# mtumalan/VisionTransformer

Measured on AMD Instinct MI355X. Metric: images/sec (512×512) ViT-B/16 seg, 1/2/4/8 MI355X + mask argmax match, higher is better.
Workload: dtype f32

## Files before the change

visiontransformer_amd/csrc/common.hpp:

```cpp
#pragma once
#include <hip/hip_runtime.h>
#include <stdint.h>

#include "../../include/vitseg.h"

namespace vitseg {

constexpr int WAVE = 64;

typedef float f32x4 __attribute__((ext_vector_type(4)));
typedef float f32x16 __attribute__((ext_vector_type(16)));
typedef short bf16x8 __attribute__((ext_vector_type(8)));
typedef short bf16x4 __attribute__((ext_vector_type(4)));

void set_error(const char* fmt, ...);
int hip_fail(hipError_t e, const char* what);

enum Opt {
    OPT_NO_F32P = 0,
    OPT_NO_P8,
    OPT_NO_H16P,
    OPT_NO_RAGGED_P8,
    OPT_NO_DROPMASK,
    OPT_DROPW_LIMIT_MB,
    OPT_UPSAMPLE_GLOBAL,
    OPT_BF16_TILES,
    OPT_F32P_NOINL,
    OPT_GN,
    OPT_NO_MASK2,
    OPT_NO_SMALL,
    OPT_SMALL_VARIANT,
    OPT_SMALL_MAX_ROWS,
    OPT_CONV_DMA,
    OPT_COUNT
};
long opt(int id);

#define VITSEG_CHECK_ARG(cond, code, ...) \
    do {                                  \
        if (!(cond)) {                    \
            ::vitseg::set_error(__VA_ARGS__); \
            return (code);                \
        }                                 \
    } while (0)

#define VITSEG_LAUNCH_CHECK(what)                               \
    do {                                                        \
        hipError_t e__ = hipGetLastError();                     \
// ... 241 lines not shown
```

visiontransformer_amd/csrc/forward.hip:

```cpp
#include "kernels.hpp"
#include "profile.hpp"
#include "forward.hpp"

namespace vitseg {

using namespace plan;

long small_max_rows() {
    const long v = opt(OPT_SMALL_MAX_ROWS);
    return v > 0 ? v : SMALL_MAX_ROWS;
}

bool small_applies(const vitseg_config* cfg, int batch, int precision) {
    Shape s;
    if (precision == VITSEG_F32X3 || opt(OPT_NO_SMALL) || check_config(cfg, &s)) return false;
    const long rows = (long)batch * s.N;
    if (!(rows < small_max_rows() && s.D % 64 == 0 && s.I % 32 == 0 && s.I > s.D && s.S % 4 == 0)) return false;
    const long lim16 = opt(OPT_SMALL_MAX_ROWS) > 0 ? opt(OPT_SMALL_MAX_ROWS) : small_max_rows_16(s.N);
    if (precision != VITSEG_F32 && !(s.I % 64 == 0 && attn_small_infer(s.Np) && rows < lim16)) return false;
    if (precision != VITSEG_F32 && ((s.D / small_splits(s.D, s.D)) % 64 || (s.I / small_splits(s.D, s.I)) % 64)) return false;
    return true;
}

namespace {
// ... 60 lines not shown
    if (!f.logits && !f.mask) return VITSEG_OK;
    const double px = (double)f.batch * s.S * s.S;
    ProfScope ps(f.prof.upsample, (f.logits ? px * s.C * 4 : 0.0) + (f.mask ? px : 0.0) + (double)f.batch * s.C * s.Np * 4, f.st);
    return launch_upsample(f.Z, f.logits, f.mask, f.batch, s.C, s.g, s.S, f.st);
}

}

int walk_large(const Fwd& f) {
    const Shape& s = f.s;
    const int Mp = f.batch * s.Np, Mt = Mp + f.batch, D = s.D, I = s.I;
    hipStream_t st = f.st;
    int rc;
    if ((rc = embed_gemm(f, f.layer(0).xin, f.h16 ? 1 : f.x3))) return rc;
    const int thin_rows = f.thin_rows ? thin_cls_rows(Mp, f.batch) : 0;
    auto gemm = [&](const void* A, int w, int b, int l, const float* R, void* C, int N, int K, int epi, int kind,
                    DropArgs dr = DropArgs{}, void* aux = nullptr) {
        GemmArgs g{};
        g.A = A; g.W = wg(f, w, l); g.bias = wt(f, b, l); g.R = R; g.C = C; g.aux = aux; g.drop = dr;
        g.M = Mt; g.N = N; g.K = K; g.lda = K; g.ldc = N;
        if (f.whole_split || thin_rows) {
            g.thin_rows = thin_rows;
            g.thin_scratch = f.scratch;
            g.thin_capacity = f.scratch_floats;
        }
        ProfScope ps(kind, 2.0 * g.M * g.N * g.K, st);
        if (f.fc1_train && epi == EPI_GELU) return launch_gemm_bf16_train(g, EPI_GELU, st);
        return f.h16 ? launch_gemm_bf16(g, A_PLAIN, epi, st, f.h16 == 2) : launch_gemm_f32(g, A_PLAIN, epi, st, f.x3);
    };
    auto lnorm = [&](const float* X, int w, int b, int l, void* H, int rows) {
        ProfScope ps(f.prof.ln, (double)rows * D * (f.h16 ? 6 : 8), st);
        return launch_layernorm(X, wt(f, w, l), wt(f, b, l), H, rows, D, f.eps, f.h16, st);
    };
    const bool mlp1 = f.prof.mlp_one_scope;
    for (int l = 0; l < s.L; ++l) {
        const LayerIO io = f.layer(l);
        if ((rc = lnorm(io.xin, VITSEG_T_LN1_W, VITSEG_T_LN1_B, l, io.h1, Mt))) return rc;
        if ((rc = gemm(io.h1, VITSEG_T_WQKV, VITSEG_T_BQKV, l, nullptr, io.qkv, 3 * D, D, EPI_BIAS, f.prof.qkv))) return rc;
        {
            ProfScope ps(f.prof.attn, 4.0 * f.batch * s.A * (double)s.N * s.N * 64, st);
            const DropArgs dr = drop(f, l, 1);
            if (io.dropw && (rc = launch_attn_dropmask((unsigned*)io.dropw, f.batch, s.Np, s.A, dr, st))) return rc;
            rc = f.h16 ? launch_attention_bf16(io.qkv, io.ctx, io.lse, f.batch, s.Np, s.A, dr, st, f.h16 == 2, io.dropw)
                       : launch_attention_f32((const float*)io.qkv, (float*)io.ctx, io.lse, f.batch, s.Np, s.A, dr, st, f.x3 != 0);
            if (rc) return rc;
        }
        if ((rc = gemm(io.ctx, VITSEG_T_WO, VITSEG_T_BO, l, io.xin, io.xmid, D, D, EPI_RESADD, f.prof.oproj, drop(f, l, 2))))
            return rc;
        if ((rc = lnorm(io.xmid, VITSEG_T_LN2_W, VITSEG_T_LN2_B, l, io.h2, Mt))) return rc;
        ProfScope ps(mlp1 ? f.prof.fc1 : -1, 4.0 * Mt * D * I, st);
        if ((rc = gemm(io.h2, VITSEG_T_W1, VITSEG_T_B1, l, nullptr, io.uact, I, D, EPI_GELU, mlp1 ? -1 : f.prof.fc1, DropArgs{},
                       io.upre)))
            return rc;
        if ((rc = gemm(io.uact, VITSEG_T_W2, VITSEG_T_B2, l, io.xmid, io.xout, D, I, EPI_RESADD, mlp1 ? -1 : f.prof.fc2,
                       drop(f, l, 3))))
            return rc;
    }
    if ((rc = lnorm(f.layer(s.L - 1).xout, VITSEG_T_LNF_W, VITSEG_T_LNF_B, 0, f.hf, Mp))) return rc;
    if ((rc = head_conv_gemm(f)) || (rc = head_1x1(f))) return rc;
    return upsample(f);
}

int walk_small(const Fwd& f) {
    const Shape& s = f.s;
    const int Mp = f.batch * s.Np, Mt = Mp + f.batch, D = s.D;
    hipStream_t st = f.st;
    float* part = f.scratch;
    const size_t dstride = (size_t)Mt * D;
    int rc;
    auto linear = [&](const void* A, int K, int w, int b, int l, void* C, int N, int epi, void* aux, int kind) {
// ... 112 lines not shown
```

visiontransformer_amd/csrc/gemm_dispatch.hip:

```cpp
#include "gemm_tiles.hpp"

namespace vitseg {
namespace {

int whole_split_shape(int M, int N, int K, int kstep) { return K % kstep == 0 ? whole_split(M, N, K, kstep) : 0; }

int thin_slices(int K, int kstep) {
    if (K < 256 || K % kstep != 0) return 0;
    const int sl = K / kstep / 4;
    return sl > THIN_MAX_SPLITS ? THIN_MAX_SPLITS : sl < 1 ? 1 : sl;
}

int whole_split_applies(const GemmArgs& a, int epi, int kstep) {
    const int sp = whole_split_shape(a.M, a.N, a.K, kstep);
    const bool ok = sp && a.thin_scratch && (size_t)sp * a.M * a.N <= a.thin_capacity && !a.drop.thresh &&
                    !a.aux && a.splitk <= 1 && a.ldc % 4 == 0 && (epi == EPI_BIAS || epi == EPI_GELU || epi == EPI_RESADD);
    return ok ? sp : 0;
}

int thin_split_applies(const GemmArgs& a, int epi, int kstep) {
    const bool h16 = kstep == 64;
    const int sl = thin_slices(a.K, kstep);
    const bool ok = sl && a.thin_scratch && a.thin_rows > 0 && a.thin_rows <= THIN_MAX_ROWS && a.M > a.thin_rows &&
                    (size_t)sl * a.thin_rows * a.N <= a.thin_capacity && (a.M - a.thin_rows) % BM == 0 &&
// ... 23 lines not shown
    int slices;
    int colsum_rows;
};

}

int launch_gemm_f32(const GemmArgs& a_in, int amode, int epi, hipStream_t s, int x3) {
    if (x3 != 1 && x3 != 2) x3 = 0;
    GemmArgs a = a_in;
    if (amode == A_PLAIN) {
        if (const int sp = whole_split_applies(a_in, epi, 32)) {
            a.thin_rows = a_in.M;
            return launch_thin_rows(GT_F32, x3, a, epi, sp, s);
        }
        if (const int sl = thin_split_applies(a_in, epi, 32)) {
            if (int rc = launch_thin_rows(GT_F32, x3, a_in, epi, sl, s)) return rc;
            a.M = a_in.M - a_in.thin_rows;
        }
    }
    a.thin_scratch = nullptr;
    VITSEG_CHECK_ARG(a.M > 0 && a.N > 0 && a.K > 0 && a.K % 4 == 0, VITSEG_EINVAL, "gemm_f32: bad M/N/K %d %d %d", a.M, a.N, a.K);
    VITSEG_CHECK_ARG(a.N % 4 == 0 && a.ldc % 4 == 0, VITSEG_ESHAPE, "gemm: N=%d and ldc=%d must be multiples of 4", a.N, a.ldc);
    if (amode == A_PLAIN) {
        VITSEG_CHECK_ARG(a.lda % 4 == 0, VITSEG_EINVAL, "gemm_f32: lda %% 4");
        if (!x3 && gemm_f32p_applies(a, epi)) return launch_gemm_f32p(a, epi, s);
    } else if (amode == A_PATCH && epi == EPI_POS) {
        VITSEG_CHECK_ARG(a.P % 4 == 0, VITSEG_ESHAPE, "patch size must be a multiple of 4");
    } else if (amode == A_CONV3 && epi == EPI_RELU) {
        VITSEG_CHECK_ARG(a.D % 4 == 0, VITSEG_ESHAPE, "hidden size must be a multiple of 4");
    }
    static const char* const who[3] = {"gemm_f32", "gemm_f32 (x3)", "gemm_f32 (x3, split W)"};
// ... 58 lines not shown
    r.body_rows = a.M;
    if (amode == A_PLAIN) {
        VITSEG_CHECK_ARG(a.lda % 8 == 0, VITSEG_EINVAL, "gemm_bf16: lda %% 8");
        r.body = xl ? HK_XL : large ? HK_LARGE : HK_TILE;
        if (epi == EPI_BIAS || epi == EPI_GELU || epi == EPI_DGELU || epi == EPI_RESADD) return VITSEG_OK;
    } else if (amode == A_CONV3 && (epi == EPI_RELU || epi == EPI_BIAS)) {
        VITSEG_CHECK_ARG(a.D % 64 == 0 && a.zeros, VITSEG_ESHAPE, "%s must be a multiple of 64",
                         epi == EPI_RELU ? "hidden size" : "channel count");
        r.body = large ? HK_LARGE : HK_TILE;
        return VITSEG_OK;
    }
    set_error("gemm_bf16: unsupported amode/epilogue %d/%d", amode, epi);
    return VITSEG_EINVAL;
}

int launch_gemm_bf16(const GemmArgs& a_in, int amode, int epi, hipStream_t s, bool f16) {
    H16Route r;
    if (int rc = route_h16(a_in, amode, epi, r)) return rc;
    const GemmType type = f16 ? GT_F16 : GT_BF16;
    const bool out_f32 = epi == EPI_RESADD || amode == A_CONV3;
    GemmArgs a = a_in;
    if (r.slices) {
        a.thin_rows = r.tail_rows;
        if (int rc = launch_thin_rows(type, 0, a, epi, r.slices, s)) return rc;
    }
    a.M = r.body_rows;
    a.thin_scratch = nullptr;
    if (!r.colsum_rows) a.colsum_scratch = nullptr;
    int rc = VITSEG_OK;
    switch (r.body) {
        case HK_NONE: break;
        case HK_P8: rc = launch_gemm_p8(a, epi, s, f16); break;
        case HK_H16P: rc = launch_gemm_h16p(a, s, f16); break;
        case HK_XL: rc = launch_gemm_large(f16, amode, epi, 256, a, s, "gemm_bf16"); break;
        case HK_LARGE: rc = launch_gemm_large(f16, amode, epi, 128, a, s, "gemm_bf16"); break;
        case HK_TILE: rc = launch_gemm_tile(type, out_f32, amode, epi, 0, a, s, "gemm_bf16");
    }
    if (rc) return rc;
    if (r.tail_rows && !r.slices) {
        GemmArgs t = a;
        const auto row = [&](const void* p, size_t esz) { return (char*)p + (size_t)r.body_rows * a.ldc * esz; };
        t.M = r.tail_rows;
        t.row_base = a.row_base + r.body_rows;
        t.A = (const char*)a.A + (size_t)r.body_rows * a.lda * 2;
        if (a.aux) t.aux = row(a.aux, 2);
        if (a.R) t.R = (const float*)row(a.R, epi == EPI_RESADD ? 4 : 2);
        t.C = row(a.C, out_f32 ? 4 : 2);
        if ((rc = launch_gemm_tile(type, out_f32, A_PLAIN, epi, 0, t, s, "gemm_bf16"))) return rc;
    }
    if (!a_in.colsum_out) return VITSEG_OK;
    VITSEG_CHECK_ARG(a_in.colsum_scratch && !f16, VITSEG_EINVAL, "gemm: column sums need bf16 + scratch");
    if (r.colsum_rows > 0)
        return launch_colsum_finish_fused((const bf16_t*)a_in.C + (size_t)r.colsum_rows * a_in.ldc, a_in.M - r.colsum_rows,
                                          2 * ((r.colsum_rows + 255) / 256), a_in.colsum_out, a_in.colsum_scratch, a_in.N,
// ... 40 lines not shown
```

visiontransformer_amd/csrc/gemm_tile.hip:

```cpp
#include "gemm_tiles.hpp"

namespace vitseg {
namespace {

template <typename T> struct Elem;
template <> struct Elem<float> { static constexpr int CE = 4, BKE = 32; };
template <> struct Elem<bf16_t> { static constexpr int CE = 8, BKE = 64; };
template <> struct Elem<f16_t> { static constexpr int CE = 8, BKE = 64; };

template <typename T>
struct ARow {
    const T* base;
    int y, x;
    bool valid;
};

template <typename T, int AMODE>
__device__ __forceinline__ ARow<T> make_arow(const GemmArgs& p, int m) {
    ARow<T> r;
    r.valid = m < p.M;
    r.y = r.x = 0;
    const T* A = (const T*)p.A;
    if (!r.valid) {
        r.base = A;
// ... 467 lines not shown
    else
        gemm_tile<T, OutT, AMODE, EPI, 2, 2, TA, TB, X3>(p, lds, m0, n0, (wave >> 1) * 64, (wave & 1) * 64);
}

template <typename T, typename OutT, int AMODE, int EPI, int TA = 0, int TB = 0, int X3 = 0>
int launch_one(GemmArgs a, hipStream_t s) {
    if (a.ldw == 0) a.ldw = TB ? a.N : a.K;
    if (!a.gn) a.gn = env_gn();
    const int tiles = ((a.M + BM - 1) / BM) * ((a.N + BN - 1) / BN);
    const int splits = a.splitk > 1 ? a.splitk : 1;
    hipLaunchKernelGGL((gemm_kernel<T, OutT, AMODE, EPI, TA, TB, X3>), dim3(tiles, splits), dim3(256), 0, s, a);
    VITSEG_LAUNCH_CHECK("gemm");
    return VITSEG_OK;
}

template <int EPI, typename OutT>
__global__ __launch_bounds__(256) void thin_reduce_kernel(const float* __restrict__ partial, const float* __restrict__ bias,
                                                          const float* __restrict__ R, OutT* __restrict__ C, int rows, int N,
                                                          int ldc, int splits, OutT* __restrict__ aux, DropArgs drop,
                                                          unsigned row0) {
    const int n4 = N >> 2;
    const int i = blockIdx.x * 256 + threadIdx.x;
    if (i >= rows * n4) return;
    const int r = i / n4, c = (i - r * n4) * 4;
    const size_t slab = (size_t)rows * N;
    f32x4 acc = *(const f32x4*)(partial + (size_t)r * N + c);
    for (int sIdx = 1; sIdx < splits; ++sIdx) {
        const f32x4 v = *(const f32x4*)(partial + sIdx * slab + (size_t)r * N + c);
#pragma unroll
        for (int e = 0; e < 4; ++e) acc[e] += v[e];
    }
    f32x4 b4 = {0.f, 0.f, 0.f, 0.f};
    if (bias) b4 = *(const f32x4*)(bias + c);
    f32x4 res = {0.f, 0.f, 0.f, 0.f};
    if (EPI == EPI_RESADD) res = *(const f32x4*)(R + (size_t)r * ldc + c);
    if constexpr (EPI == EPI_DGELU) {
        const uint2 d = *(const uint2*)((const OutT*)R + (size_t)r * ldc + c);
        res[0] = H16<OutT>::lo(d.x);
        res[1] = H16<OutT>::hi(d.x);
        res[2] = H16<OutT>::lo(d.y);
        res[3] = H16<OutT>::hi(d.y);
    }
    f32x4 der = {0.f, 0.f, 0.f, 0.f};
    const unsigned key = drop.thresh ? drop_key(drop.seed, drop.stream, row0 + (unsigned)r) : 0u;
#pragma unroll
    for (int e = 0; e < 4; ++e) {
// ... 13 lines not shown
    if constexpr (sizeof(OutT) == 4) {
        *(f32x4*)(C + (size_t)r * ldc + c) = acc;
    } else {
        uint2 h;
        h.x = H16<OutT>::pack2(acc[0], acc[1]);
        h.y = H16<OutT>::pack2(acc[2], acc[3]);
        *(uint2*)(C + (size_t)r * ldc + c) = h;
        if (EPI == EPI_GELU && aux) {
            h.x = H16<OutT>::pack2(der[0], der[1]);
            h.y = H16<OutT>::pack2(der[2], der[3]);
            *(uint2*)(aux + (size_t)r * ldc + c) = h;
        }
    }
}

template <typename OutT>
int launch_thin_reduce(const GemmArgs& a, int epi, int splits, hipStream_t s) {
    const int rows = a.thin_rows, body = a.M - rows;
    const int blocks = (rows * (a.N / 4) + 255) / 256;
    const float* R = nullptr;
    if (a.R) R = epi == EPI_DGELU ? (const float*)((const OutT*)a.R + (size_t)body * a.ldc) : a.R + (size_t)body * a.ldc;
    OutT* C = (OutT*)a.C + (size_t)body * a.ldc;
    OutT* aux = a.aux ? (OutT*)a.aux + (size_t)body * a.ldc : nullptr;
    const unsigned row0 = (unsigned)(a.row_base + body);
#define VITSEG_THIN(E)                                                                                                 \
    hipLaunchKernelGGL((thin_reduce_kernel<E, OutT>), dim3(blocks), dim3(256), 0, s, a.thin_scratch, a.bias, R, C, rows, \
                       a.N, a.ldc, splits, aux, a.drop, row0)
    switch (epi) {
        case EPI_BIAS: VITSEG_THIN(EPI_BIAS); break;
        case EPI_GELU: VITSEG_THIN(EPI_GELU); break;
        case EPI_DGELU:
            if constexpr (sizeof(OutT) == 4) {
                set_error("thin_reduce: dGELU epilogue is 16-bit only");
                return VITSEG_EINVAL;
            } else {
                VITSEG_THIN(EPI_DGELU);
            }
            break;
        default: VITSEG_THIN(EPI_RESADD);
    }
#undef VITSEG_THIN
    VITSEG_LAUNCH_CHECK("thin_reduce");
    return VITSEG_OK;
}

}

int launch_gemm_tile(GemmType type, bool out_f32, int amode, int epi, int x3, const GemmArgs& a, hipStream_t s, const char* who) {
#define ROW(ID, T, OutT, AMODE, EPI, X3) \
    if (type == ID && out_f32 == (sizeof(OutT) == 4) && amode == AMODE && epi == EPI && x3 == X3) return launch_one<T, OutT, AMODE, EPI, 0, 0, X3>(a, s);
#define ROW_X3(AMODE, EPI) ROW(GT_F32, float, float, AMODE, EPI, 0) ROW(GT_F32, float, float, AMODE, EPI, 1) ROW(GT_F32, float, float, AMODE, EPI, 2)
#define ROW_H16(AMODE, EPI) ROW(GT_BF16, bf16_t, bf16_t, AMODE, EPI, 0) ROW(GT_F16, f16_t, f16_t, AMODE, EPI, 0)
#define ROW_H16_F32(AMODE, EPI) ROW(GT_BF16, bf16_t, float, AMODE, EPI, 0) ROW(GT_F16, f16_t, float, AMODE, EPI, 0)
    ROW_X3(A_PLAIN, EPI_BIAS) ROW_X3(A_PLAIN, EPI_GELU) ROW_X3(A_PLAIN, EPI_RESADD) ROW(GT_F32, float, float, A_PLAIN, EPI_RELU, 0)
    ROW_X3(A_PATCH, EPI_POS) ROW_X3(A_CONV3, EPI_RELU)
    ROW_H16(A_PLAIN, EPI_BIAS) ROW_H16(A_PLAIN, EPI_GELU) ROW_H16(A_PLAIN, EPI_DGELU)
    ROW_H16_F32(A_PLAIN, EPI_RESADD) ROW_H16_F32(A_PLAIN, EPI_BIAS) ROW_H16_F32(A_CONV3, EPI_RELU) ROW_H16_F32(A_CONV3, EPI_BIAS)
// ... 18 lines not shown
    const int rows = a.thin_rows, body = a.M - rows;
    GemmArgs t = a;
    t.A = (const char*)a.A + (size_t)body * a.lda * (type == GT_F32 ? 4 : 2);
    t.M = rows;
    t.bias = nullptr;
    t.R = nullptr;
    t.C = a.thin_scratch;
    t.ldc = a.N;
    t.splitk = slices;
    t.split_stride = (size_t)rows * a.N;
    t.thin_scratch = nullptr;
    if (type != GT_F32) {
        t.aux = nullptr;
        t.drop = DropArgs{};
    }
    if (int rc = launch_gemm_tile(type, true, A_PLAIN, EPI_BIAS, x3, t, s, "gemm (K slices)")) return rc;
    if (type == GT_F32 || epi == EPI_RESADD) return launch_thin_reduce<float>(a, epi, slices, s);
    return type == GT_F16 ? launch_thin_reduce<f16_t>(a, epi, slices, s) : launch_thin_reduce<bf16_t>(a, epi, slices, s);
}

}
```

visiontransformer_amd/csrc/kernels.hpp:

```cpp
#pragma once
#include "common.hpp"

namespace vitseg {

enum AMode {
    A_PLAIN = 0,
    A_PATCH = 1,
    A_CONV3 = 2
};
enum Epi {
    EPI_BIAS = 0,
    EPI_GELU = 1,
    EPI_RESADD = 2,
    EPI_RELU = 3,
    EPI_POS = 4,
    EPI_DGELU = 5
};

struct GemmArgs {
    const void* A;
    const void* W;
    const float* bias;
    const float* R;
    void* C;
    int M, N, K;
    int lda, ldc;
    int ldw;
    void* aux;
    float* colsum_out;
    float* colsum_scratch;
    int S, P, g, Np, Cin, D;
    const void* zeros;
    int splitk;
    size_t split_stride;
    float* thin_scratch;
    size_t thin_capacity;
    int thin_rows;
    int gn;
    DropArgs drop;
    int row_base;
};

constexpr int THIN_MAX_SPLITS = 16, THIN_MAX_ROWS = 64;
inline size_t thin_scratch_floats(int max_n) { return (size_t)THIN_MAX_SPLITS * THIN_MAX_ROWS * max_n; }
inline int whole_split(int M, int N, int K, int kstep) {
    const int tiles = ((M + 127) / 128) * ((N + 127) / 128);
    if (tiles > 128 || K < 512) return 0;
    int s = K / kstep / 4;
    if (s > 8) s = 8;
    return s >= 2 ? s : 0;
}
int launch_gemm_f32(const GemmArgs& a, int amode, int epi, hipStream_t s, int x3 = 0);
int launch_gemm_f32_bwd(const GemmArgs& a, int amode, int ta, int tb, int epi, hipStream_t s);
size_t wgrad_scratch_floats(int M, int N, int K);
int launch_wgrad_f32(GemmArgs a, float* scratch, hipStream_t s);
int launch_wgrad_bf16_tt(GemmArgs a, float* scratch, hipStream_t s);
int launch_gemm_bf16_train(const GemmArgs& a, int epi, hipStream_t s);
size_t wgrad_bf16_scratch_floats(int M, int N, int K);
int wgrad_bf16_splits(int M, int N, int K, bool p8);
// ... 76 lines not shown
```

visiontransformer_amd/csrc/vitseg_api.hip:

```cpp
#include <ctype.h>
#include <stdarg.h>
#include <stdio.h>
#include <stdlib.h>
#include <strings.h>

#include <atomic>

#include <vector>

#include "kernels.hpp"
#include "profile.hpp"
#include "forward.hpp"

namespace vitseg {

static thread_local char g_err[512] = "";

void set_error(const char* fmt, ...) {
    va_list ap;
    va_start(ap, fmt);
    vsnprintf(g_err, sizeof(g_err), fmt, ap);
    va_end(ap);
}

int hip_fail(hipError_t e, const char* what) {
    set_error("%s: %s", what, hipGetErrorString(e));
    return VITSEG_EHIP;
}

static const char* const g_opt_names[OPT_COUNT] = {"no_f32p", "no_p8", "no_h16p", "no_ragged_p8", "no_dropmask",
                                                   "dropw_limit_mb", "upsample_global", "bf16_tiles", "f32p_noinl", "gn", "no_mask2", "no_small",
                                                   "small_variant", "small_max_rows", "conv_dma"};
static std::atomic<long> g_opts[OPT_COUNT];
static int opt_index(const char* name) {
    if (!name) return -1;
    for (int i = 0; i < OPT_COUNT; ++i)
        if (!strcasecmp(name, g_opt_names[i])) return i;
    return -1;
}
static long opt_parse(int id, const char* text) {
    if (id == OPT_BF16_TILES && (text[0] == 's' || text[0] == 'l' || text[0] == 'x')) return text[0] == 's' ? 1 : text[0] == 'l' ? 2 : 3;
    char* end = nullptr;
    const long v = strtol(text, &end, 10);
    if (end != text) return v;
    return (id == OPT_DROPW_LIMIT_MB || id == OPT_GN || id == OPT_SMALL_VARIANT || id == OPT_SMALL_MAX_ROWS || id == OPT_BF16_TILES) ? 0 : 1;
}
static const bool g_opts_loaded = [] {
// ... 334 lines not shown
                            int N, int K, int epilogue, int f16, int thin_rows, float* scratch, size_t scratch_floats,
                            float dropout_p, uint32_t dropout_seed, uint32_t dropout_stream, float* colsum_out,
                            float* colsum_scratch, void* stream) {
    VITSEG_CHECK_ARG(A && Wt && C, VITSEG_EINVAL, "linear_h16_ex: null pointer");
    VITSEG_CHECK_ARG(epilogue == EPI_BIAS || epilogue == EPI_GELU || epilogue == EPI_RESADD || epilogue == EPI_DGELU,
                     VITSEG_EINVAL, "linear_h16_ex: epilogue %d", epilogue);
    VITSEG_CHECK_ARG((epilogue != EPI_RESADD && epilogue != EPI_DGELU) || R, VITSEG_EINVAL, "linear_h16_ex: epilogue needs R");
    VITSEG_CHECK_ARG(dropout_p >= 0.f && dropout_p < 1.f, VITSEG_EINVAL, "linear_h16_ex: dropout_p %f", dropout_p);
    GemmArgs g{};
    g.A = A; g.W = Wt; g.bias = bias; g.R = (const float*)R; g.C = C; g.aux = aux;
    g.M = M; g.N = N; g.K = K; g.lda = K; g.ldc = N;
    if (thin_rows > 0) {
        g.thin_rows = thin_rows;
        g.thin_scratch = scratch;
        g.thin_capacity = scratch_floats;
    }
    g.drop = drop_args(dropout_p, dropout_seed, dropout_stream);
    VITSEG_CHECK_ARG(!colsum_out || (colsum_scratch && epilogue == EPI_DGELU && !f16), VITSEG_EINVAL,
                     "linear_h16_ex: column sums come with the bf16 dGELU epilogue and need scratch");
    g.colsum_out = colsum_out;
    g.colsum_scratch = colsum_out ? colsum_scratch : nullptr;
    return launch_gemm_bf16(g, A_PLAIN, epilogue, (hipStream_t)stream, f16 != 0);
}

size_t vitseg_op_colsum_scratch_floats(int M, int N) { return colsum_scratch_floats(M, N); }

size_t vitseg_op_wgrad_bf16_scratch_floats(int M, int N, int K) { return wgrad_bf16_scratch_floats(M, N, K); }

int vitseg_op_wgrad_bf16(const void* dY, const void* X, float* dW, float* scratch, const void* zeros, int M, int N, int K,
                         void* stream) {
// ... 10 lines not shown
                              float dropout_p, uint32_t dropout_seed, uint32_t dropout_stream, void* stream) {
    VITSEG_CHECK_ARG(A && Wt && C, VITSEG_EINVAL, "linear_f32_thin: null pointer");
    VITSEG_CHECK_ARG(epilogue >= 0 && epilogue <= (x3 ? 2 : 3), VITSEG_EINVAL, "linear_f32_thin: epilogue %d", epilogue);
    VITSEG_CHECK_ARG(epilogue != EPI_RESADD || R, VITSEG_EINVAL, "linear_f32_thin: residual epilogue needs R");
    VITSEG_CHECK_ARG(x3 == 0 || x3 == 1, VITSEG_EINVAL, "linear_f32_thin: x3 %d", x3);
    VITSEG_CHECK_ARG(dropout_p >= 0.f && dropout_p < 1.f, VITSEG_EINVAL, "linear_f32_thin: dropout_p %f", dropout_p);
    VITSEG_CHECK_ARG(!aux || epilogue == EPI_GELU, VITSEG_EINVAL, "linear_f32_thin: aux belongs to the GELU epilogue");
    VITSEG_CHECK_ARG(thin_rows >= 0, VITSEG_EINVAL, "linear_f32_thin: thin_rows %d", thin_rows);
    GemmArgs g{};
    g.A = A; g.W = Wt; g.bias = bias; g.R = R; g.C = C; g.aux = aux;
    g.M = M; g.N = N; g.K = K; g.lda = K; g.ldc = N;
    if (scratch && scratch_floats) {
        g.thin_rows = thin_rows;
        g.thin_scratch = scratch;
        g.thin_capacity = scratch_floats;
    }
    if (epilogue == EPI_RESADD) g.drop = drop_args(dropout_p, dropout_seed, dropout_stream);
    return launch_gemm_f32(g, A_PLAIN, epilogue, (hipStream_t)stream, x3);
}

size_t vitseg_op_wgrad_f32_scratch_floats(int M, int N, int K) { return M > 0 && N > 0 && K > 0 ? wgrad_scratch_floats(M, N, K) : 0; }

int vitseg_op_wgrad_f32(const float* dY, const float* X, float* dW, float* scratch, int M, int N, int K, void* stream) {
    VITSEG_CHECK_ARG(dY && X && dW, VITSEG_EINVAL, "wgrad_f32: null pointer");
    GemmArgs g{};
    g.A = dY; g.W = X; g.C = dW;
    g.M = M; g.N = N; g.K = K; g.lda = M; g.ldw = N; g.ldc = N;
    return launch_wgrad_f32(g, scratch, (hipStream_t)stream);
}

// ... 218 lines not shown
```

visiontransformer_amd/csrc/vitseg_train.hip:

```cpp
#include <stdlib.h>

#include <mutex>

#include "kernels.hpp"
#include "profile.hpp"
#include "forward.hpp"

using namespace vitseg;
using namespace vitseg::plan;

namespace {

struct LayerBufs {
    size_t xin, h1, qkv, ctx, lse, xmid, h2, upre, uact;
    size_t dropw;
};
constexpr size_t DROPW_KEEP_LIMIT = (size_t)4 << 30;
struct TrainPlan {
    size_t Mt, Mp;
    size_t layer0, layer_stride;
    LayerBufs lb;
    size_t xfinal, hf, f, z;
    size_t dxa, dxb, dh, dqkv, du, dctx, dvec, g, dz, df, t, wd, scratch, wscratch, ce_partial, total;
    size_t wscratch_floats;
    size_t dxc, wt, zero, dhf, Kpad;
    size_t wt_all, wt_layer;
    size_t dxm;
    size_t dropw_shared;
    bool dropw_per_layer;
    size_t pos, dpos, dpos_t;
};

TrainPlan make_train_plan(const Shape& s, int B, int precision, int g0) {
    TrainPlan p{};
    p.Mp = (size_t)B * s.Np;
    p.Mt = p.Mp + B;
    const bool lp = precision == VITSEG_BF16;
    const size_t act = lp ? 2 : 4;
    const size_t MtD = p.Mt * s.D * 4, MtI = p.Mt * (size_t)s.I * 4;
// ... 68 lines not shown
        p.dxc = take(dxc_n * 2);
        p.dhf = take(p.Mp * s.D * 4);
        p.wt = take(wide * s.D * 2);
        p.wt_layer = (size_t)s.D * (3 * s.D + s.D + 2 * (size_t)s.I);
        p.wt_all = take(p.wt_layer * s.L * 2);
        p.zero = take(256);
        size_t w = wgrad_bf16_scratch_floats(s.D, s.I, (int)p.Kpad);
        auto mx = [&](size_t v) { w = v > w ? v : w; };
        mx(wgrad_bf16_scratch_floats(s.I, s.D, (int)p.Kpad));
        mx(wgrad_bf16_scratch_floats(s.D, s.D, (int)p.Kpad));
        mx(wgrad_bf16_scratch_floats(3 * s.D, s.D, (int)p.Kpad));
        mx(wgrad_scratch_floats(MID, 9 * s.D, (int)p.Mp));
        mx(wgrad_scratch_floats(s.D, s.Kp, (int)p.Mp));
        mx(wgrad_bf16_scratch_floats(MID, 9 * s.D, (int)p.Mp));
        mx(wgrad_bf16_scratch_floats(s.D, s.Kp, (int)p.Mp));
        mx(thin_scratch_floats(s.I > 3 * s.D ? s.I : 3 * s.D));
        p.wscratch = take(w * 4);
        p.wscratch_floats = w;
    }
    if (g0 != s.g) {
        p.pos = take((size_t)s.N * s.D * 4);
        p.dpos = take((size_t)s.N * s.D * 4);
        p.dpos_t = take((size_t)s.g * g0 * s.D * 4);
    }
    p.total = off;
    return p;
}

struct Ctx {
    void* const* events = nullptr;
// ... 279 lines not shown
        };
}

void route_bf16(const Ctx& c, BwdRoute& r) {
    const Shape s = c.s;
    const int Mt = (int)c.p.Mt, Mp = (int)c.p.Mp, D = s.D, I = s.I, B = c.B;
    hipStream_t st = c.st;
    float *scratch = c.T(c.p.scratch), *wscr = c.T(c.p.wscratch);
    void *dXc = c.TV(c.p.dxc), *t = c.TV(c.p.t);
    auto tt = [=, &c](const void* dY, const void* X, float* dW, int M, int Nd, int Kd) {
        GemmArgs g = lin(dY, X, nullptr, nullptr, dW, Nd, Kd, M, Nd, Kd);
        g.ldw = Kd;
        g.zeros = c.ws + c.p.zero;
        return launch_wgrad_bf16_tt(g, wscr, st);
    };
    r.prepare = [=, &c] {
        const size_t src0[4] = {tensor_offset(c.lay, VITSEG_T_WQKV, 0), tensor_offset(c.lay, VITSEG_T_WO, 0),
                                tensor_offset(c.lay, VITSEG_T_W1, 0), tensor_offset(c.lay, VITSEG_T_W2, 0)};
        const int R4[4] = {3 * D, D, I, D}, C4[4] = {D, D, D, I};
        ProfScope ps(VITSEG_K_TRAIN_DGRAD, 0.0, st);
        return launch_transpose_layers_bf16(c.params_lp, c.TV(c.p.wt_all), src0, R4, C4, c.lay.layer_stride, s.L, st);
    };
    r.head_wgrad = [=, &c](float* dW) {
        if (int rc = launch_cast_bf16(c.T(c.p.df), dXc, (size_t)Mp * MID, st)) return rc;
        if (int rc = launch_im2col3x3_bf16(c.TV(c.p.hf), t, B, s.g, D, st)) return rc;
        return tt(dXc, t, dW, Mp, MID, 9 * D);
    };
    r.head_dgrad = [=, &c] {
        float* dHf = c.T(c.p.dhf);
        if (int rc = launch_cast_bf16(c.T(c.p.wd), c.TV(c.p.wt), (size_t)D * 9 * MID, st)) return dense(rc, nullptr);
        GemmArgs g = lin(dXc, c.TV(c.p.wt), nullptr, nullptr, dHf, Mp, D, 9 * MID, 0, D);
// ... 19 lines not shown
    r.wgrad = [=](const void* dY, const void* X, float* dW, int M, int Nd, int Kd) {
        ProfScope ps(VITSEG_K_TRAIN_WGRAD, 2.0 * M * Nd * Kd, st);
        return tt(dY, X, dW, M, Nd, Kd);
    };
    r.dgrad = [=, &c](const void* dY, int wt, int l, void* dX, int Nd, int Kd, int epi, const void* R, float* bias_grad, bool) {
        const size_t DD = (size_t)D * D;
        const size_t off = wt == VITSEG_T_WQKV ? 0 : wt == VITSEG_T_WO ? 3 * DD : wt == VITSEG_T_W1 ? 4 * DD : 4 * DD + (size_t)I * D;
        ProfScope ps(VITSEG_K_TRAIN_DGRAD, 2.0 * Mt * Nd * Kd, st);
        GemmArgs g = lin(dY, (const unsigned short*)c.TV(c.p.wt_all) + (size_t)l * c.p.wt_layer + off, nullptr, (const float*)R, dX,
                         Mt, Kd, Nd, Nd, Kd);
        g.ldw = Nd;
        if (thin_cls_rows(Mp, B)) {
            g.thin_rows = B;
            g.thin_scratch = wscr;
            g.thin_capacity = c.p.wscratch_floats;
        }
        g.colsum_out = bias_grad;
        g.colsum_scratch = bias_grad ? scratch : nullptr;
        return dense(launch_gemm_bf16_train(g, epi, st), dX);
    };
    r.attn_bwd = [=, &c](int l, const void* dCTX, void* dQKV, float* bias_grad) {
        ProfScope ps(VITSEG_K_TRAIN_ATTN_BWD, attn_flops(c, 10), st);
        if (c.dropw(l) && !c.p.dropw_per_layer)
            if (int rc = launch_attn_dropmask((unsigned*)c.dropw(l), B, s.Np, s.A, c.dr(l, 1), st)) return rc;
        return launch_attention_bwd_bf16(c.LV(l, c.p.lb.qkv), c.LV(l, c.p.lb.ctx), dCTX, c.L(l, c.p.lb.lse), c.T(c.p.dvec), dQKV,
                                         B, s.Np, s.A, c.dr(l, 1), st, c.dropw(l), bias_grad);
    };
    r.patch_wgrad = [=, &c](const float* x, float* dX, float* dW) {
        if (s.Kp % 8 == 0) {
            if (int rc = launch_cast_bf16(dX, dXc, (size_t)Mp * D, st)) return rc;
// ... 216 lines not shown
```

Baseline: 612.4.

## Fuse thin-row split-K GEMM with last-block reduction and skip unread CLS rows

```diff
diff --git a/visiontransformer_amd/csrc/common.hpp b/visiontransformer_amd/csrc/common.hpp
--- a/visiontransformer_amd/csrc/common.hpp
+++ b/visiontransformer_amd/csrc/common.hpp
@@ -32,6 +32,7 @@
     OPT_SMALL_VARIANT,
     OPT_SMALL_MAX_ROWS,
     OPT_CONV_DMA,
+    OPT_THIN_MODE,
     OPT_COUNT
 };
 long opt(int id);
diff --git a/visiontransformer_amd/csrc/forward.hip b/visiontransformer_amd/csrc/forward.hip
--- a/visiontransformer_amd/csrc/forward.hip
+++ b/visiontransformer_amd/csrc/forward.hip
@@ -98,8 +98,12 @@
     int rc;
     if ((rc = embed_gemm(f, f.layer(0).xin, f.h16 ? 1 : f.x3))) return rc;
     const int thin_rows = f.thin_rows ? thin_cls_rows(Mp, f.batch) : 0;
+    int thin_counters = 0;
+    if ((f.whole_split || thin_rows) && (rc = thin_counters_reset(f.scratch, f.scratch_floats, st, &thin_counters))) return rc;
+    const LayerIO io_last = f.layer(s.L - 1);
+    const bool skip_cls = thin_rows && !f.fc1_train && !io_last.lse && !io_last.upre && f.drop_p == 0.f && !(opt(OPT_THIN_MODE) & 2);
     auto gemm = [&](const void* A, int w, int b, int l, const float* R, void* C, int N, int K, int epi, int kind,
-                    DropArgs dr = DropArgs{}, void* aux = nullptr) {
+                    DropArgs dr = DropArgs{}, void* aux = nullptr, bool cls_unread = false) {
         GemmArgs g{};
         g.A = A; g.W = wg(f, w, l); g.bias = wt(f, b, l); g.R = R; g.C = C; g.aux = aux; g.drop = dr;
         g.M = Mt; g.N = N; g.K = K; g.lda = K; g.ldc = N;
@@ -107,6 +111,8 @@
             g.thin_rows = thin_rows;
             g.thin_scratch = f.scratch;
             g.thin_capacity = f.scratch_floats;
+            g.thin_counters = thin_counters;
+            g.skip_rows = cls_unread ? thin_rows : 0;
         }
         ProfScope ps(kind, 2.0 * g.M * g.N * g.K, st);
         if (f.fc1_train && epi == EPI_GELU) return launch_gemm_bf16_train(g, EPI_GELU, st);
@@ -119,6 +125,7 @@
     const bool mlp1 = f.prof.mlp_one_scope;
     for (int l = 0; l < s.L; ++l) {
         const LayerIO io = f.layer(l);
+        const bool skip = skip_cls && l == s.L - 1;
         if ((rc = lnorm(io.xin, VITSEG_T_LN1_W, VITSEG_T_LN1_B, l, io.h1, Mt))) return rc;
         if ((rc = gemm(io.h1, VITSEG_T_WQKV, VITSEG_T_BQKV, l, nullptr, io.qkv, 3 * D, D, EPI_BIAS, f.prof.qkv))) return rc;
         {
@@ -129,15 +136,16 @@
                        : launch_attention_f32((const float*)io.qkv, (float*)io.ctx, io.lse, f.batch, s.Np, s.A, dr, st, f.x3 != 0);
             if (rc) return rc;
         }
-        if ((rc = gemm(io.ctx, VITSEG_T_WO, VITSEG_T_BO, l, io.xin, io.xmid, D, D, EPI_RESADD, f.prof.oproj, drop(f, l, 2))))
-            return rc;
-        if ((rc = lnorm(io.xmid, VITSEG_T_LN2_W, VITSEG_T_LN2_B, l, io.h2, Mt))) return rc;
+        if ((rc = gemm(io.ctx, VITSEG_T_WO, VITSEG_T_BO, l, io.xin, io.xmid, D, D, EPI_RESADD, f.prof.oproj, drop(f, l, 2),
+                       nullptr, skip)))
+            return rc;
+        if ((rc = lnorm(io.xmid, VITSEG_T_LN2_W, VITSEG_T_LN2_B, l, io.h2, skip ? Mp : Mt))) return rc;
         ProfScope ps(mlp1 ? f.prof.fc1 : -1, 4.0 * Mt * D * I, st);
         if ((rc = gemm(io.h2, VITSEG_T_W1, VITSEG_T_B1, l, nullptr, io.uact, I, D, EPI_GELU, mlp1 ? -1 : f.prof.fc1, DropArgs{},
-                       io.upre)))
+                       io.upre, skip)))
             return rc;
         if ((rc = gemm(io.uact, VITSEG_T_W2, VITSEG_T_B2, l, io.xmid, io.xout, D, I, EPI_RESADD, mlp1 ? -1 : f.prof.fc2,
-                       drop(f, l, 3))))
+                       drop(f, l, 3), nullptr, skip)))
             return rc;
     }
     if ((rc = lnorm(f.layer(s.L - 1).xout, VITSEG_T_LNF_W, VITSEG_T_LNF_B, 0, f.hf, Mp))) return rc;
diff --git a/visiontransformer_amd/csrc/gemm_dispatch.hip b/visiontransformer_amd/csrc/gemm_dispatch.hip
--- a/visiontransformer_amd/csrc/gemm_dispatch.hip
+++ b/visiontransformer_amd/csrc/gemm_dispatch.hip
@@ -61,7 +61,8 @@
             return launch_thin_rows(GT_F32, x3, a, epi, sp, s);
         }
         if (const int sl = thin_split_applies(a_in, epi, 32)) {
-            if (int rc = launch_thin_rows(GT_F32, x3, a_in, epi, sl, s)) return rc;
+            if (a_in.skip_rows != a_in.thin_rows)
+                if (int rc = launch_thin_rows(GT_F32, x3, a_in, epi, sl, s)) return rc;
             a.M = a_in.M - a_in.thin_rows;
         }
     }
@@ -150,13 +151,22 @@
     return VITSEG_EINVAL;
 }
 
+int thin_counters_reset(float* scratch, size_t capacity, hipStream_t s, int* lent) {
+    unsigned* cnt = (opt(OPT_THIN_MODE) & 1) ? nullptr : thin_counters_at(scratch, capacity);
+    *lent = cnt ? 1 : 0;
+    if (!cnt) return VITSEG_OK;
+    const hipError_t e = hipMemsetAsync(cnt, 0, THIN_COUNTER_WORDS * sizeof(unsigned), s);
+    return e == hipSuccess ? VITSEG_OK : hip_fail(e, "hipMemsetAsync(thin counters)");
+}
+
 int launch_gemm_bf16(const GemmArgs& a_in, int amode, int epi, hipStream_t s, bool f16) {
     H16Route r;
     if (int rc = route_h16(a_in, amode, epi, r)) return rc;
     const GemmType type = f16 ? GT_F16 : GT_BF16;
     const bool out_f32 = epi == EPI_RESADD || amode == A_CONV3;
     GemmArgs a = a_in;
-    if (r.slices) {
+    const bool skip_tail = r.body != HK_NONE && r.tail_rows > 0 && a_in.skip_rows == r.tail_rows;
+    if (r.slices && !skip_tail) {
         a.thin_rows = r.tail_rows;
         if (int rc = launch_thin_rows(type, 0, a, epi, r.slices, s)) return rc;
     }
@@ -173,7 +183,7 @@
         case HK_TILE: rc = launch_gemm_tile(type, out_f32, amode, epi, 0, a, s, "gemm_bf16");
     }
     if (rc) return rc;
-    if (r.tail_rows && !r.slices) {
+    if (r.tail_rows && !r.slices && !skip_tail) {
         GemmArgs t = a;
         const auto row = [&](const void* p, size_t esz) { return (char*)p + (size_t)r.body_rows * a.ldc * esz; };
         t.M = r.tail_rows;
diff --git a/visiontransformer_amd/csrc/gemm_tile.hip b/visiontransformer_amd/csrc/gemm_tile.hip
--- a/visiontransformer_amd/csrc/gemm_tile.hip
+++ b/visiontransformer_amd/csrc/gemm_tile.hip
@@ -505,22 +505,33 @@
     return VITSEG_OK;
 }
 
+template <int NJ>
+__device__ __forceinline__ void thin_sum(const float* partial, size_t slab, int splits, const size_t (&off)[NJ], f32x4 (&acc)[NJ]) {
+#pragma unroll
+    for (int j = 0; j < NJ; ++j) acc[j] = *(const f32x4*)(partial + off[j]);
+    for (int s0 = 1; s0 < splits; s0 += 8) {
+        f32x4 v[8][NJ];
+#pragma unroll
+        for (int u = 0; u < 8; ++u) {
+            const size_t so = (size_t)min(s0 + u, splits - 1) * slab;
+#pragma unroll
+            for (int j = 0; j < NJ; ++j) v[u][j] = *(const f32x4*)(partial + so + off[j]);
+        }
+#pragma unroll
+        for (int u = 0; u < 8; ++u) {
+            if (s0 + u < splits) {
+#pragma unroll
+                for (int j = 0; j < NJ; ++j)
+#pragma unroll
+                    for (int e = 0; e < 4; ++e) acc[j][e] += v[u][j][e];
+            }
+        }
+    }
+}
+
 template <int EPI, typename OutT>
-__global__ __launch_bounds__(256) void thin_reduce_kernel(const float* __restrict__ partial, const float* __restrict__ bias,
-                                                          const float* __restrict__ R, OutT* __restrict__ C, int rows, int N,
-                                                          int ldc, int splits, OutT* __restrict__ aux, DropArgs drop,
-                                                          unsigned row0) {
-    const int n4 = N >> 2;
-    const int i = blockIdx.x * 256 + threadIdx.x;
-    if (i >= rows * n4) return;
-    const int r = i / n4, c = (i - r * n4) * 4;
-    const size_t slab = (size_t)rows * N;
-    f32x4 acc = *(const f32x4*)(partial + (size_t)r * N + c);
-    for (int sIdx = 1; sIdx < splits; ++sIdx) {
-        const f32x4 v = *(const f32x4*)(partial + sIdx * slab + (size_t)r * N + c);
-#pragma unroll
-        for (int e = 0; e < 4; ++e) acc[e] += v[e];
-    }
+__device__ __forceinline__ void thin_epilogue(f32x4 acc, const float* bias, const float* R, OutT* C, int ldc, OutT* aux,
+                                              const DropArgs& drop, unsigned row0, int r, int c) {
     f32x4 b4 = {0.f, 0.f, 0.f, 0.f};
     if (bias) b4 = *(const f32x4*)(bias + c);
     f32x4 res = {0.f, 0.f, 0.f, 0.f};
@@ -564,18 +575,52 @@
     }
 }
 
+template <int EPI, typename OutT>
+__global__ __launch_bounds__(256) void thin_reduce_kernel(const float* __restrict__ partial, const float* __restrict__ bias,
+                                                          const float* __restrict__ R, OutT* __restrict__ C, int rows, int N,
+                                                          int ldc, int splits, OutT* __restrict__ aux, DropArgs drop,
+                                                          unsigned row0) {
+    const int n4 = N >> 2;
+    const int i = blockIdx.x * 256 + threadIdx.x;
+    if (i >= rows * n4) return;
+    const int r = i / n4, c = (i - r * n4) * 4;
+    const size_t off[1] = {(size_t)r * N + c};
+    f32x4 acc[1];
+    thin_sum<1>(partial, (size_t)rows * N, splits, off, acc);
+    thin_epilogue<EPI, OutT>(acc[0], bias, R, C, ldc, aux, drop, row0, r, c);
+}
+
+struct ThinEpi {
+    const float* bias;
+    const void* R;
+    void* C;
+    void* aux;
+    int rows, N, ldc, splits;
+    DropArgs drop;
+    unsigned row0;
+};
+
+template <typename OutT>
+ThinEpi thin_epi(const GemmArgs& a, int epi, int splits) {
+    const int rows = a.thin_rows, body = a.M - rows;
+    ThinEpi q{};
+    q.bias = a.bias;
+    if (a.R) q.R = epi == EPI_DGELU ? (const void*)((const OutT*)a.R + (size_t)body * a.ldc) : (const void*)(a.R + (size_t)body * a.ldc);
+    q.C = (OutT*)a.C + (size_t)body * a.ldc;
+    q.aux = a.aux ? (OutT*)a.aux + (size_t)body * a.ldc : nullptr;
+    q.rows = rows; q.N = a.N; q.ldc = a.ldc; q.splits = splits;
+    q.drop = a.drop;
+    q.row0 = (unsigned)(a.row_base + body);
+    return q;
+}
+
 template <typename OutT>
 int launch_thin_reduce(const GemmArgs& a, int epi, int splits, hipStream_t s) {
-    const int rows = a.thin_rows, body = a.M - rows;
-    const int blocks = (rows * (a.N / 4) + 255) / 256;
-    const float* R = nullptr;
-    if (a.R) R = epi == EPI_DGELU ? (const float*)((const OutT*)a.R + (size_t)body * a.ldc) : a.R + (size_t)body * a.ldc;
-    OutT* C = (OutT*)a.C + (size_t)body * a.ldc;
-    OutT* aux = a.aux ? (OutT*)a.aux + (size_t)body * a.ldc : nullptr;
-    const unsigned row0 = (unsigned)(a.row_base + body);
-#define VITSEG_THIN(E)                                                                                                 \
-    hipLaunchKernelGGL((thin_reduce_kernel<E, OutT>), dim3(blocks), dim3(256), 0, s, a.thin_scratch, a.bias, R, C, rows, \
-                       a.N, a.ldc, splits, aux, a.drop, row0)
+    const ThinEpi q = thin_epi<OutT>(a, epi, splits);
+    const int blocks = (q.rows * (a.N / 4) + 255) / 256;
+#define VITSEG_THIN(E)                                                                                                        \
+    hipLaunchKernelGGL((thin_reduce_kernel<E, OutT>), dim3(blocks), dim3(256), 0, s, a.thin_scratch, q.bias, (const float*)q.R, \
+                       (OutT*)q.C, q.rows, q.N, q.ldc, splits, (OutT*)q.aux, q.drop, q.row0)
     switch (epi) {
         case EPI_BIAS: VITSEG_THIN(EPI_BIAS); break;
         case EPI_GELU: VITSEG_THIN(EPI_GELU); break;
@@ -591,6 +636,83 @@
     }
 #undef VITSEG_THIN
     VITSEG_LAUNCH_CHECK("thin_reduce");
+    return VITSEG_OK;
+}
+
+template <int EPI, typename OutT>
+__device__ __forceinline__ void thin_reduce_tile(const float* partial, const ThinEpi& q, int m0, int n0) {
+    const int rows_t = min(BM, q.rows - m0), c4n = min(BN, q.N - n0) >> 2;
+    const int n = rows_t * c4n;
+    const size_t slab = (size_t)q.rows * q.N;
+    for (int base = 0; base < n; base += 4 * 256) {
+        int r[4], c[4];
+        size_t off[4];
+        f32x4 acc[4];
+#pragma unroll
+        for (int j = 0; j < 4; ++j) {
+            const int i = min(base + j * 256 + (int)threadIdx.x, n - 1);
+            r[j] = m0 + i / c4n;
+            c[j] = n0 + (i - (i / c4n) * c4n) * 4;
+            off[j] = (size_t)r[j] * q.N + c[j];
+        }
+        thin_sum<4>(partial, slab, q.splits, off, acc);
+#pragma unroll
+        for (int j = 0; j < 4; ++j)
+            if (base + j * 256 + (int)threadIdx.x < n)
+                thin_epilogue<EPI, OutT>(acc[j], q.bias, (const float*)q.R, (OutT*)q.C, q.ldc, (OutT*)q.aux, q.drop, q.row0, r[j], c[j]);
+    }
+}
+
+template <typename T, int X3>
+__global__ __launch_bounds__(256, 2) void thin_fused_kernel(const GemmArgs p, const ThinEpi q, unsigned* cnt, int epi) {
+    __shared__ __attribute__((aligned(16))) float lds[2][2][BM * BKF];
+    const int wave = threadIdx.x >> 6;
+    const int tiles_n = (p.N + BN - 1) / BN;
+    const int tile = blockIdx.x, tile_m = tile / tiles_n, tile_n = tile - tile_m * tiles_n;
+    const int m0 = tile_m * BM, n0 = tile_n * BN;
+    const int rows_valid = p.M - m0;
+    if (rows_valid <= 32)
+        gemm_tile<T, float, A_PLAIN, EPI_BIAS, 1, 1, 0, 0, X3>(p, lds, m0, n0, 0, wave * 32);
+    else if (rows_valid <= 64)
+        gemm_tile<T, float, A_PLAIN, EPI_BIAS, 2, 1, 0, 0, X3>(p, lds, m0, n0, 0, wave * 32);
+    else
+        gemm_tile<T, float, A_PLAIN, EPI_BIAS, 2, 2, 0, 0, X3>(p, lds, m0, n0, (wave >> 1) * 64, (wave & 1) * 64);
+
+    asm volatile("s_waitcnt vmcnt(0)" ::: "memory");
+    __syncthreads();
+    volatile unsigned* last = (volatile unsigned*)&lds[0][0][0];
+    if (threadIdx.x == 0) {
+        __builtin_amdgcn_fence(__ATOMIC_RELEASE, "agent");
+        asm volatile("s_waitcnt vmcnt(0)" ::: "memory");
+        const unsigned seen = __hip_atomic_fetch_add(cnt + tile, 1u, __ATOMIC_RELAXED, __HIP_MEMORY_SCOPE_AGENT);
+        const bool is_last = seen == gridDim.y - 1;
+        if (is_last) {
+            __hip_atomic_store(cnt + tile, 0u, __ATOMIC_RELAXED, __HIP_MEMORY_SCOPE_AGENT);
+            __builtin_amdgcn_fence(__ATOMIC_ACQUIRE, "agent");
+            asm volatile("s_waitcnt vmcnt(0)" ::: "memory");
+        }
+        *last = is_last ? 1u : 0u;
+    }
+    __syncthreads();
+    if (!*last) return;
+    const float* partial = (const float*)p.C;
+    if constexpr (sizeof(T) == 4) {
+        if (epi == EPI_GELU) thin_reduce_tile<EPI_GELU, float>(partial, q, m0, n0);
+        else if (epi == EPI_RESADD) thin_reduce_tile<EPI_RESADD, float>(partial, q, m0, n0);
+        else thin_reduce_tile<EPI_BIAS, float>(partial, q, m0, n0);
+    } else {
+        if (epi == EPI_GELU) thin_reduce_tile<EPI_GELU, T>(partial, q, m0, n0);
+        else if (epi == EPI_DGELU) thin_reduce_tile<EPI_DGELU, T>(partial, q, m0, n0);
+        else if (epi == EPI_RESADD) thin_reduce_tile<EPI_RESADD, float>(partial, q, m0, n0);
+        else thin_reduce_tile<EPI_BIAS, T>(partial, q, m0, n0);
+    }
+}
+
+template <typename T, int X3>
+int launch_thin_fused(GemmArgs t, const ThinEpi& q, unsigned* cnt, int epi, int tiles, hipStream_t s) {
+    if (t.ldw == 0) t.ldw = t.K;
+    hipLaunchKernelGGL((thin_fused_kernel<T, X3>), dim3(tiles, t.splitk), dim3(256), 0, s, t, q, cnt, epi);
+    VITSEG_LAUNCH_CHECK("thin_fused");
     return VITSEG_OK;
 }
 
@@ -639,9 +761,29 @@
         t.aux = nullptr;
         t.drop = DropArgs{};
     }
+    const int tiles = ((rows + BM - 1) / BM) * ((a.N + BN - 1) / BN);
+    const bool f32_out = type == GT_F32 || epi == EPI_RESADD;
+    unsigned* cnt = a.thin_counters ? thin_counters_at(a.thin_scratch, a.thin_capacity) : nullptr;
+    if (cnt && !(opt(OPT_THIN_MODE) & 1) && tiles <= THIN_COUNTER_WORDS && a.K % (type == GT_F32 ? 4 : 64) == 0 &&
+        (float*)cnt >= a.thin_scratch + (size_t)slices * rows * a.N &&
+        (epi == EPI_BIAS || epi == EPI_GELU || epi == EPI_RESADD || (type != GT_F32 && epi == EPI_DGELU))) {
+        const ThinEpi q = f32_out ? thin_epi<float>(a, epi, slices)
+                                  : type == GT_F16 ? thin_epi<f16_t>(a, epi, slices) : thin_epi<bf16_t>(a, epi, slices);
+        if (type == GT_BF16) return launch_thin_fused<bf16_t, 0>(t, q, cnt, epi, tiles, s);
+        if (type == GT_F16) return launch_thin_fused<f16_t, 0>(t, q, cnt, epi, tiles, s);
+        if (x3 == 1) return launch_thin_fused<float, 1>(t, q, cnt, epi, tiles, s);
+        if (x3 == 2) return launch_thin_fused<float, 2>(t, q, cnt, epi, tiles, s);
+        return launch_thin_fused<float, 0>(t, q, cnt, epi, tiles, s);
+    }
     if (int rc = launch_gemm_tile(type, true, A_PLAIN, EPI_BIAS, x3, t, s, "gemm (K slices)")) return rc;
-    if (type == GT_F32 || epi == EPI_RESADD) return launch_thin_reduce<float>(a, epi, slices, s);
-    return type == GT_F16 ? launch_thin_reduce<f16_t>(a, epi, slices, s) : launch_thin_reduce<bf16_t>(a, epi, slices, s);
-}
-
-}
+    if (int rc = f32_out ? launch_thin_reduce<float>(a, epi, slices, s)
+                         : type == GT_F16 ? launch_thin_reduce<f16_t>(a, epi, slices, s) : launch_thin_reduce<bf16_t>(a, epi, slices, s))
+        return rc;
+    if (cnt && (float*)cnt < a.thin_scratch + (size_t)slices * rows * a.N) {
+        const hipError_t e = hipMemsetAsync(cnt, 0, THIN_COUNTER_WORDS * sizeof(unsigned), s);
+        if (e != hipSuccess) return hip_fail(e, "hipMemsetAsync(thin counters)");
+    }
+    return VITSEG_OK;
+}
+
+}
diff --git a/visiontransformer_amd/csrc/kernels.hpp b/visiontransformer_amd/csrc/kernels.hpp
--- a/visiontransformer_amd/csrc/kernels.hpp
+++ b/visiontransformer_amd/csrc/kernels.hpp
@@ -32,6 +32,7 @@
     int S, P, g, Np, Cin, D;
     const void* zeros;
     int splitk;
+    int thin_counters;
     size_t split_stride;
     float* thin_scratch;
     size_t thin_capacity;
@@ -39,10 +40,16 @@
     int gn;
     DropArgs drop;
     int row_base;
+    int skip_rows;
 };
 
 constexpr int THIN_MAX_SPLITS = 16, THIN_MAX_ROWS = 64;
 inline size_t thin_scratch_floats(int max_n) { return (size_t)THIN_MAX_SPLITS * THIN_MAX_ROWS * max_n; }
+constexpr int THIN_COUNTER_WORDS = 128;
+inline unsigned* thin_counters_at(float* scratch, size_t capacity) {
+    return scratch && capacity > (size_t)THIN_COUNTER_WORDS ? (unsigned*)(scratch + capacity) - THIN_COUNTER_WORDS : nullptr;
+}
+int thin_counters_reset(float* scratch, size_t capacity, hipStream_t s, int* lent);
 inline int whole_split(int M, int N, int K, int kstep) {
     const int tiles = ((M + 127) / 128) * ((N + 127) / 128);
     if (tiles > 128 || K < 512) return 0;
diff --git a/visiontransformer_amd/csrc/vitseg_api.hip b/visiontransformer_amd/csrc/vitseg_api.hip
--- a/visiontransformer_amd/csrc/vitseg_api.hip
+++ b/visiontransformer_amd/csrc/vitseg_api.hip
@@ -30,7 +30,7 @@
 
 static const char* const g_opt_names[OPT_COUNT] = {"no_f32p", "no_p8", "no_h16p", "no_ragged_p8", "no_dropmask",
                                                    "dropw_limit_mb", "upsample_global", "bf16_tiles", "f32p_noinl", "gn", "no_mask2", "no_small",
-                                                   "small_variant", "small_max_rows", "conv_dma"};
+                                                   "small_variant", "small_max_rows", "conv_dma", "thin_mode"};
 static std::atomic<long> g_opts[OPT_COUNT];
 static int opt_index(const char* name) {
     if (!name) return -1;
@@ -395,6 +395,8 @@
         g.thin_rows = thin_rows;
         g.thin_scratch = scratch;
         g.thin_capacity = scratch_floats;
+        if (opt(OPT_THIN_MODE) & 4)
+            if (int rc = thin_counters_reset(scratch, scratch_floats, (hipStream_t)stream, &g.thin_counters)) return rc;
     }
     g.drop = drop_args(dropout_p, dropout_seed, dropout_stream);
     VITSEG_CHECK_ARG(!colsum_out || (colsum_scratch && epilogue == EPI_DGELU && !f16), VITSEG_EINVAL,
@@ -435,6 +437,8 @@
         g.thin_rows = thin_rows;
         g.thin_scratch = scratch;
         g.thin_capacity = scratch_floats;
+        if (opt(OPT_THIN_MODE) & 4)
+            if (int rc = thin_counters_reset(scratch, scratch_floats, (hipStream_t)stream, &g.thin_counters)) return rc;
     }
     if (epilogue == EPI_RESADD) g.drop = drop_args(dropout_p, dropout_seed, dropout_stream);
     return launch_gemm_f32(g, A_PLAIN, epilogue, (hipStream_t)stream, x3);
diff --git a/visiontransformer_amd/csrc/vitseg_train.hip b/visiontransformer_amd/csrc/vitseg_train.hip
--- a/visiontransformer_amd/csrc/vitseg_train.hip
+++ b/visiontransformer_amd/csrc/vitseg_train.hip
@@ -23,6 +23,7 @@
     size_t xfinal, hf, f, z;
     size_t dxa, dxb, dh, dqkv, du, dctx, dvec, g, dz, df, t, wd, scratch, wscratch, ce_partial, total;
     size_t wscratch_floats;
+    size_t wgrad_floats;
     size_t dxc, wt, zero, dhf, Kpad;
     size_t wt_all, wt_layer;
     size_t dxm;
@@ -121,6 +122,7 @@
         mx(wgrad_scratch_floats(s.D, s.Kp, (int)p.Mp));
         mx(wgrad_bf16_scratch_floats(MID, 9 * s.D, (int)p.Mp));
         mx(wgrad_bf16_scratch_floats(s.D, s.Kp, (int)p.Mp));
+        p.wgrad_floats = w;
         mx(thin_scratch_floats(s.I > 3 * s.D ? s.I : 3 * s.D));
         p.wscratch = take(w * 4);
         p.wscratch_floats = w;
@@ -430,7 +432,11 @@
         g.zeros = c.ws + c.p.zero;
         return launch_wgrad_bf16_tt(g, wscr, st);
     };
+    const bool cnt_room = c.p.wgrad_floats + THIN_COUNTER_WORDS <= c.p.wscratch_floats;
     r.prepare = [=, &c] {
+        int cnt = 0;
+        if (cnt_room)
+            if (int rc = thin_counters_reset(wscr, c.p.wscratch_floats, st, &cnt)) return rc;
         const size_t src0[4] = {tensor_offset(c.lay, VITSEG_T_WQKV, 0), tensor_offset(c.lay, VITSEG_T_WO, 0),
                                 tensor_offset(c.lay, VITSEG_T_W1, 0), tensor_offset(c.lay, VITSEG_T_W2, 0)};
         const int R4[4] = {3 * D, D, I, D}, C4[4] = {D, D, D, I};
@@ -480,6 +486,7 @@
             g.thin_rows = B;
             g.thin_scratch = wscr;
             g.thin_capacity = c.p.wscratch_floats;
+            g.thin_counters = cnt_room;
         }
         g.colsum_out = bias_grad;
         g.colsum_scratch = bias_grad ? scratch : nullptr;
```

After: 609.4. No clear change (-0.5%).
